# Etschbeijer/GibbsSampling

Measured on NVIDIA B200. Metric: gibbs_window_scores_per_sec, higher is better.
Workload: dtype f64

## Files before the change

### gibbssampling_b200/_abi.py

```python
from __future__ import annotations

import ctypes as C
import os

from . import _build

GIBBS_OK = 0
GIBBS_ERR_ARG = 1
GIBBS_ERR_SYMBOL = 2
GIBBS_ERR_SHORT_SEQ = 3
GIBBS_ERR_CUDA = 4
GIBBS_ERR_NCCL = 5
GIBBS_ERR_NOMEM = 6
GIBBS_ERR_ROULETTE = 7
GIBBS_ERR_UNSUPPORTED = 8

GIBBS_SITE_SAMPLER = 0
GIBBS_MOTIF_SAMPLER = 1
GIBBS_RNG_PHILOX = 0
GIBBS_RNG_INJECTED = 1
GIBBS_BG_FIXED = 0
GIBBS_BG_DATA = 1
GIBBS_MAX_K = 32
PHASE_INIT, PHASE_GREEDY, PHASE_LEFT, PHASE_RIGHT, PHASE_STOCHASTIC, PHASE_MOTIF_GREEDY = 1, 2, 4, 8, 16, 32

EXPORTS = [
    "gibbs_abi_version", "gibbs_last_error", "gibbs_device_count", "gibbs_create", "gibbs_upload",
    "gibbs_destroy", "gibbs_set_stream", "gibbs_num_sequences", "gibbs_set_team_warps", "gibbs_synchronize",
    "gibbs_loo_counts", "gibbs_window_scores", "gibbs_pick_argmax", "gibbs_pick_roulette",
    "gibbs_set_start_ppm", "gibbs_set_start_state", "gibbs_run_device", "gibbs_fetch", "gibbs_run", "gibbs_device_results",
    "gibbs_host_alloc", "gibbs_host_free", "gibbs_measure_smem_bandwidth",
    "gibbs_set_option", "gibbs_fetch_best", "gibbs_fetch_positions", "gibbs_fetch_best_positions",
    "gibbs_set_start_motif_state",
    "gibbs_multi_create", "gibbs_multi_destroy", "gibbs_multi_num_devices", "gibbs_multi_handle",
    "gibbs_multi_run_device", "gibbs_multi_fetch_best",
    "gibbs_batch_create", "gibbs_batch_destroy", "gibbs_batch_run_device", "gibbs_batch_fetch", "gibbs_batch_fetch_best",
]
GIBBS_OPT_INIT_PATH, GIBBS_OPT_EXACT_SCANS, GIBBS_OPT_STAGE2_AT, GIBBS_OPT_STAGE3_AT, GIBBS_OPT_CLUSTER, GIBBS_OPT_MIN_WIDTH = 1, 2, 3, 4, 5, 6
GIBBS_OPT_TILE_ROWS = 7
GIBBS_OPT_SEQ_SWEEPS = 8
GIBBS_INIT_AUTO, GIBBS_INIT_CHAIN, GIBBS_INIT_WIDE, GIBBS_INIT_SMEM, GIBBS_INIT_TILED = 0, 1, 2, 3, 4


class GibbsError(RuntimeError):

    def __init__(self, code: int, msg: str):
        super().__init__(f"[gibbs_status {code}] {msg}")
        self.code = code


class GibbsArgumentError(GibbsError, ValueError):
    """ArgumentNullException / ArgumentException of the reference (fs:24, fs:183)."""


class GibbsSymbolError(GibbsError, IndexError):
    """IndexOutOfRangeException analogue: a symbol the 2-bit tables cannot index (fs:17)."""


class GibbsShortSequenceError(GibbsError, ValueError):
    """InvalidOperationException from Array.take when a sequence is shorter than k (fs:152)."""


class GibbsCudaError(GibbsError):
# ... 126 lines not shown
```

### gibbssampling_b200/csrc/gibbs_api.cu

```cuda
#include "../../include/gibbs_b200.h"
#include "gibbs_kernels.cuh"
#include "gibbs_motif.cuh"
#include "gibbs_motif2.cuh"
#include "gibbs_drift.cuh"
#include "gibbs_batch.cuh"

#include <algorithm>
#include <cmath>
#include <cstdarg>
#include <cstdio>
#include <cstdlib>
#include <cstring>
#include <new>
#include <vector>

namespace gibbs {
#define GIBBS_CHAIN_TU(name) cudaError_t name(const ChainArgs &a, int grid, int smem, cudaStream_t stream)
GIBBS_CHAIN_TU(launch_chain_t1);
GIBBS_CHAIN_TU(launch_chain_t4);
GIBBS_CHAIN_TU(launch_chain_t8);
GIBBS_CHAIN_TU(launch_chain_t16);
GIBBS_CHAIN_TU(launch_chain_masked_t1);
GIBBS_CHAIN_TU(launch_chain_masked_t4);
GIBBS_CHAIN_TU(launch_chain_masked_drift_t1);
// ... 131 lines not shown
    DevBuf<double> start_ppm;
    int32_t start_ppm_k = 0;
    DevBuf<int32_t> basecnt, maskcnt;
    DevBuf<int32_t> ss;
    bool ss_valid = false;
    bool drift_valid = false;
    double drift_pc = 0;
    int32_t drift_alen = 0;
    int32_t gcnt[4] = {0, 0, 0, 0};
    DevBuf<int32_t> ctl, resume, pending;
    int32_t run_extra_launches = 0;
    int32_t team_warps = 0;
    int32_t run_team = 0;
    int sm_count = 0;
    std::vector<int32_t> len_host;
    int32_t start_max_excess = 0;
    int32_t opt_init_path = 0;
    int32_t opt_exact_scans = 0;
    int32_t opt_stage2_at = 4, opt_stage3_at = 1;
    int32_t opt_min_width = -1;
    int32_t opt_seq_sweeps = 1;
    int32_t opt_tile_rows = 0;
    int32_t opt_cluster = 8;
    int32_t cluster_cap[2] = {-1, -1};
    int32_t cluster_cap_n = 0, cluster_cap_rw = 0, cluster_cap_k = 0;
    int32_t run_stages = 0;
    int32_t wt_span = 0, drift_span = 0;
    DevBuf<int32_t> pos2;
    DevBuf<double> sc2;
    int32_t run_m = 1;
    int32_t start_m = 0;
    bool best_valid = false;
    int32_t run_init_path = 0;
    DevBuf<int32_t> win_sites;
    DevBuf<double> win_scores;
    size_t smem_optin = 0;
};

namespace {

int32_t set_device(const gibbs_handle *h) {
    CUDA_TRY(cudaSetDevice(h->device));
    return GIBBS_OK;
}

int32_t check_params(const gibbs_handle *h, const gibbs_params *p) {
    if (!h) return fail(GIBBS_ERR_ARG, "null handle");
    if (!p) return fail(GIBBS_ERR_ARG, "null params");
    if (h->n < 1) return fail(GIBBS_ERR_ARG, "handle holds no sequences");
    if (p->k < 1 || p->k > GIBBS_MAX_K) return fail(GIBBS_ERR_ARG, "motif width k=%d outside 1..%d", p->k, GIBBS_MAX_K);
    if (h->min_len < p->k)
        return fail(GIBBS_ERR_SHORT_SEQ, "a sequence of length %d is shorter than k=%d (Array.take, fs:152)", h->min_len, p->k);
    if (p->alphabet_size < 1) return fail(GIBBS_ERR_ARG, "alphabet_size must be >= 1");
    if (!(p->pseudocount >= 0.0)) return fail(GIBBS_ERR_ARG, "pseudocount must be >= 0");
    if (p->background != GIBBS_BG_FIXED && p->background != GIBBS_BG_DATA) return fail(GIBBS_ERR_ARG, "unknown background mode %d", p->background);
    if (h->has_gap && p->alphabet_size >= 5)
        return fail(GIBBS_ERR_UNSUPPORTED, "sequences hold Gap '-' and alphabet_size = %d includes it: a fifth PWM row is not built "
                                           "(pass alphabet_size = 4 to score Gap like any other non-alphabet symbol)", p->alphabet_size);
    if (p->background == GIBBS_BG_FIXED)
// ... 144 lines not shown
        b.from_list = 0;
        b.pause_below = 0;
        cudaError_t e;
        if (masked && drift) e = team == 4 ? launch_chain_init_masked_drift_t4(b, a.n_chains, smem, h->stream) : launch_chain_init_masked_drift_t1(b, a.n_chains, smem, h->stream);
        else if (masked) e = team == 4 ? launch_chain_init_masked_t4(b, a.n_chains, smem, h->stream) : launch_chain_init_masked_t1(b, a.n_chains, smem, h->stream);
        else if (drift) e = team == 4 ? launch_chain_init_drift_t4(b, a.n_chains, smem, h->stream) : launch_chain_init_drift_t1(b, a.n_chains, smem, h->stream);
        else e = team == 4 ? launch_chain_init_t4(b, a.n_chains, smem, h->stream) : launch_chain_init_t1(b, a.n_chains, smem, h->stream);
        CUDA_TRY(e);
        a.phase_mask &= ~GIBBS_PHASE_INIT;
        h->run_extra_launches += 1;
    }
    return GIBBS_OK;
}

int32_t launch_random_starts_any(gibbs_handle *h, ChainArgs &a, bool drift) {
    switch ((a.k + 1) / 2) {
#define X(KPV) case KPV: return launch_random_starts<KPV>(h, a, drift);
        KP_CASES(X)
#undef X
    default: return fail(GIBBS_ERR_ARG, "unsupported k");
    }
}

template <int KPV>
int32_t launch_chain_kp(gibbs_handle *h, ChainArgs a, bool drift) {
    h->run_extra_launches = 0;
    const bool masked = a.s.mask != nullptr;
    {
        const int32_t rc = launch_random_starts<KPV>(h, a, drift);
        if (rc) return rc;
    }
    const int N = a.s.n, sms = h->sm_count;
    auto fits = [&](int t) { return N >= t && team_smem_bytes(a.s.row_words, t) <= 200 * 1024; };
    struct Stage { int team, pause_below, cluster, min_sweeps; };
    Stage stages[8] = {};
    int n_stages = 0;
    if (masked) {
        stages[n_stages++] = {team_smem_bytes(a.s.row_words, 4) <= 200 * 1024 ? 4 : 1, 0, 0};
    } else if (drift) {
        const int forced = h->team_warps == 16 ? 8 : h->team_warps;
        if (forced != 0) {
            stages[n_stages++] = {forced, 0, 0};
        } else {
            int first = a.n_chains > 2 * sms ? 4 : 8;
            if (first == 8 && !fits(8)) first = 4;
            if (first == 4 && !fits(4)) first = 1;
// ... 25 lines not shown
            if (h->cluster_cap_n != N || h->cluster_cap_rw != a.s.row_words || h->cluster_cap_k != a.k) {
                h->cluster_cap[0] = h->cluster_cap[1] = 0;
                int cap = 0;
                if (launch_chain_cluster4_smem(N, a.s.row_words) <= h->smem_optin &&
                    launch_chain_cluster4(a, 1, h->stream, &cap) == cudaSuccess) h->cluster_cap[0] = cap;
                cap = 0;
                if (launch_chain_cluster8_smem(N, a.s.row_words) <= h->smem_optin &&
                    launch_chain_cluster8(a, 1, h->stream, &cap) == cudaSuccess) h->cluster_cap[1] = cap;
                cudaGetLastError();
                h->cluster_cap_n = N; h->cluster_cap_rw = a.s.row_words; h->cluster_cap_k = a.k;
            }
            if (h->cluster_cap[0] > 0) {
                stages[n_stages - 1].pause_below = h->cluster_cap[0];
                stages[n_stages++] = {16, 0, 4};
                if (h->opt_cluster >= 8 && h->cluster_cap[1] > 0 && h->cluster_cap[1] < h->cluster_cap[0]) {
                    stages[n_stages - 1].pause_below = h->cluster_cap[1];
                    stages[n_stages++] = {16, 0, 8};
                }
            }
        }
    }
    h->run_team = stages[0].team == 1 && n_stages > 1 && stages[0].pause_below == a.n_chains ? 4 : stages[0].team;
    h->run_stages = n_stages;
    CUDA_TRY(h->ctl.reserve(8));
    const int32_t ctl0[8] = {a.n_chains, 0, 0, 0, 0, 0, 0, 0};
    CUDA_TRY(cudaMemcpyAsync(h->ctl.p, ctl0, sizeof ctl0, cudaMemcpyHostToDevice, h->stream));
    a.active = h->ctl.p;
    if (n_stages > 1) {
        CUDA_TRY(h->resume.reserve((size_t)a.n_chains));
        CUDA_TRY(h->pending.reserve((size_t)(n_stages - 1) * (size_t)a.n_chains));
        a.resume = h->resume.p;
    }
    for (int st = 0; st < n_stages; ++st) {
        ChainArgs b = a;
        b.pause_below = stages[st].pause_below;
        b.pause_min_sweeps = stages[st].min_sweeps;
        b.from_list = st > 0;
        {
            const int per_sm = st == 0 ? (a.n_chains + sms - 1) / sms : (stages[st - 1].pause_below + sms - 1) / sms;
            const bool seq_stage = stages[0].team == 1 && stages[0].min_sweeps > 0;
            b.min_width = stages[st].cluster ? stages[st].cluster * 16 : per_sm <= 1 ? stages[st].team
                          : h->opt_min_width >= 1 ? h->opt_min_width : seq_stage ? stages[st].team : 1;
        }
        b.pending_in = st > 0 ? h->pending.p + (size_t)(st - 1) * a.n_chains : nullptr;
        b.pending_in_n = st > 0 ? h->ctl.p + st : nullptr;
        b.pending_out = st + 1 < n_stages ? h->pending.p + (size_t)st * a.n_chains : nullptr;
        b.pending_out_n = st + 1 < n_stages ? h->ctl.p + st + 1 : nullptr;
        const int grid = st == 0 ? a.n_chains : stages[st - 1].pause_below;
        if (stages[st].cluster) {
            CUDA_TRY(stages[st].cluster == 4 ? launch_chain_cluster4(b, grid, h->stream, nullptr) : launch_chain_cluster8(b, grid, h->stream, nullptr));
        } else {
            int32_t rc = launch_team(h, stages[st].team, masked, drift, b, grid);
            if (rc) return rc;
        }
        if (st > 0) h->run_extra_launches += 1;
    }
    return GIBBS_OK;
}

int32_t launch_chain(gibbs_handle *h, const ChainArgs &a, bool drift = false) {
    const int kp = (a.k + 1) / 2;
    switch (kp) {
#define X(KPV) case KPV: return launch_chain_kp<KPV>(h, a, drift);
        KP_CASES(X)
#undef X
    default: return fail(GIBBS_ERR_ARG, "unsupported k");
    }
}

int32_t launch_loo_counts(gibbs_handle *h, const PrimArgs &a) {
    const int kp = (a.k + 1) / 2;
// ... 354 lines not shown
    if (!out) return fail(GIBBS_ERR_ARG, "null out pointer");
    *out = nullptr;
    int ndev = 0;
    cudaError_t e = cudaGetDeviceCount(&ndev);
    if (e != cudaSuccess || ndev < 1) {
        cudaGetLastError();
        return fail(GIBBS_ERR_CUDA, "no CUDA device available (%s); libgibbs_b200 has no CPU fallback",
                    e != cudaSuccess ? cudaGetErrorString(e) : "device count 0");
    }
    if (device < 0 || device >= ndev) return fail(GIBBS_ERR_ARG, "device %d outside 0..%d", device, ndev - 1);
    gibbs_handle *h = new (std::nothrow) gibbs_handle();
    if (!h) return fail(GIBBS_ERR_NOMEM, "host allocation failed");
    h->device = device;
    int32_t rc = set_device(h);
    if (!rc) {
        cudaError_t e2 = cudaStreamCreateWithFlags(&h->stream, cudaStreamNonBlocking);
        if (e2 == cudaSuccess) e2 = cudaEventCreate(&h->ev0);
        if (e2 == cudaSuccess) e2 = cudaEventCreate(&h->ev1);
        if (e2 != cudaSuccess) rc = fail(GIBBS_ERR_CUDA, "stream/event creation: %s", cudaGetErrorString(e2));
        h->own_stream = true;
    }
    if (!rc) {
        cudaError_t e3 = cudaDeviceGetAttribute(&h->sm_count, cudaDevAttrMultiProcessorCount, device);
        int optin = 0;
        if (e3 == cudaSuccess) e3 = cudaDeviceGetAttribute(&optin, cudaDevAttrMaxSharedMemoryPerBlockOptin, device);
        if (e3 != cudaSuccess) rc = fail(GIBBS_ERR_CUDA, "device attribute: %s", cudaGetErrorString(e3));
        h->smem_optin = (size_t)(optin > 0 ? optin : 0);
    }
    if (!rc) rc = upload(h, seqs, offsets, n_seqs);
    if (rc) {
        gibbs_destroy(h);
        return rc;
    }
    *out = h;
    return GIBBS_OK;
}

int32_t gibbs_upload(gibbs_handle *h, const uint8_t *seqs, const int64_t *offsets, int32_t n_seqs) {
    if (!h) return fail(GIBBS_ERR_ARG, "null handle");
    return upload(h, seqs, offsets, n_seqs);
}

int32_t gibbs_destroy(gibbs_handle *h) {
    if (!h) return GIBBS_OK;
    cudaSetDevice(h->device);
    if (h->stream) cudaStreamSynchronize(h->stream);
    h->ascii.release(); h->off.release(); h->packed.release(); h->len.release(); h->flags.release();
    h->mask.release(); h->rowflag.release(); h->symflags.release(); h->wide.release();
    h->wtab.release(); h->prim_sites.release(); h->prim_i32.release(); h->prim_f64.release();
    h->sites.release(); h->hv.release(); h->scores.release(); h->sums.release(); h->uniforms.release();
// ... 589 lines not shown
        if (counts_out) memset(counts_out, 0, (size_t)h->run_k * 4 * sizeof(int32_t));
    }
    if (n_out) *n_out = best < 0 ? 1 : N;
    if (sum_out) *sum_out = sum;
    if (restart_out) *restart_out = best;
    if (stats_out) {
        float ms = 0.f;
        CUDA_TRY(cudaEventElapsedTime(&ms, h->ev0, h->ev1));
        stats_out->site_updates = (int64_t)st[ST_SITE_UPDATES];
        stats_out->window_scores = (int64_t)st[ST_WINDOW_SCORES];
        stats_out->sweeps = (int64_t)st[ST_SWEEPS];
        stats_out->exact_rescans = (int64_t)st[ST_EXACT_RESCANS];
        stats_out->capped_chains = (int64_t)st[ST_CAPPED];
        stats_out->speculative_discards = (int64_t)st[ST_SPECULATED];
        stats_out->kernel_launches = h->run_launches + extra_launches;
        stats_out->fast_path = h->run_fast;
        stats_out->team_warps = h->run_team;
        stats_out->init_path = h->run_init_path;
        stats_out->kernel_ms = (double)ms;
    }
    return GIBBS_OK;
}

int32_t gibbs_set_option(gibbs_handle *h, int32_t option, int32_t value) {
    if (!h) return fail(GIBBS_ERR_ARG, "null handle");
    switch (option) {
    case GIBBS_OPT_INIT_PATH:
        if (value < GIBBS_INIT_AUTO || value > GIBBS_INIT_TILED) return fail(GIBBS_ERR_ARG, "GIBBS_OPT_INIT_PATH takes GIBBS_INIT_AUTO .. GIBBS_INIT_TILED");
        h->opt_init_path = value;
        return GIBBS_OK;
    case GIBBS_OPT_EXACT_SCANS:
        h->opt_exact_scans = value != 0;
        return GIBBS_OK;
    case GIBBS_OPT_MIN_WIDTH:
        if (value < -1 || value > 128) return fail(GIBBS_ERR_ARG, "GIBBS_OPT_MIN_WIDTH takes -1 (automatic) .. 128");
        h->opt_min_width = value;
        return GIBBS_OK;
    case GIBBS_OPT_SEQ_SWEEPS:
        if (value < 0 || value > 3) return fail(GIBBS_ERR_ARG, "GIBBS_OPT_SEQ_SWEEPS takes 0 .. 3");
        h->opt_seq_sweeps = value;
        return GIBBS_OK;
    case GIBBS_OPT_TILE_ROWS:
        if (value < 0) return fail(GIBBS_ERR_ARG, "GIBBS_OPT_TILE_ROWS takes 0 (what fits) or a positive number of sequences");
        h->opt_tile_rows = value;
        return GIBBS_OK;
    case GIBBS_OPT_CLUSTER:
        if (value != 0 && value != 4 && value != 8) return fail(GIBBS_ERR_ARG, "GIBBS_OPT_CLUSTER takes 0, 4 or 8");
        h->opt_cluster = value;
        return GIBBS_OK;
    case GIBBS_OPT_STAGE2_AT:
    case GIBBS_OPT_STAGE3_AT:
        if (value < 1 || value > 16) return fail(GIBBS_ERR_ARG, "hand-over thresholds are 1 .. 16 chains per SM");
        (option == GIBBS_OPT_STAGE2_AT ? h->opt_stage2_at : h->opt_stage3_at) = value;
        if (h->opt_stage3_at > h->opt_stage2_at) h->opt_stage3_at = h->opt_stage2_at;
        return GIBBS_OK;
    default:
        return fail(GIBBS_ERR_ARG, "unknown option %d", option);
    }
}

int32_t gibbs_run(gibbs_handle *h, const gibbs_params *p, int32_t n_chains, int64_t chain_id_base, uint64_t seed,
                  int32_t rng_mode, const double *uniforms, int64_t uniforms_per_chain, int32_t *sites_out,
                  double *scores_out, double *sums_out, int32_t *best_chain_out, int32_t *counts_out,
                  gibbs_run_stats *stats_out) {
    int32_t rc = gibbs_run_device(h, p, n_chains, chain_id_base, seed, rng_mode, uniforms, uniforms_per_chain);
    if (rc) return rc;
    return gibbs_fetch(h, sites_out, scores_out, sums_out, best_chain_out, counts_out, stats_out);
}

struct gibbs_multi {
    std::vector<gibbs_handle *> dev;
// ... 667 lines not shown
```

### gibbssampling_b200/csrc/gibbs_batch.cuh

```cuda
#pragma once
#include "gibbs_kernels.cuh"

namespace gibbs {

struct BatchTable {
    const ChainArgs *sets;
    const int32_t *set_ids;
    const int32_t *chain_off;
    int32_t n;
};

#ifndef GIBBS_BATCH_T4_MIN_BLOCKS
#define GIBBS_BATCH_T4_MIN_BLOCKS 6
#endif
#ifndef GIBBS_BATCH_T4_DRIFT_MIN_BLOCKS
#define GIBBS_BATCH_T4_DRIFT_MIN_BLOCKS 5
#endif
#define GIBBS_BATCH_MIN_BLOCKS(T, DRIFT, INIT_ONLY) \
    (INIT_ONLY ? (T == 1 ? 8 : 4) : T == 1 ? 16 : DRIFT ? GIBBS_BATCH_T4_DRIFT_MIN_BLOCKS : GIBBS_BATCH_T4_MIN_BLOCKS)

template <int KP, int T, bool MASKED, bool DRIFT, bool INIT_ONLY>
static __global__ void __launch_bounds__(32 * T, GIBBS_BATCH_MIN_BLOCKS(T, DRIFT, INIT_ONLY)) chain_batch_kernel(const ChainArgs run, const BatchTable bt) {
    extern __shared__ __align__(128) unsigned char smem_raw[];
    constexpr int THREADS = 32 * T;
// ... 5 lines not shown
        const int g = blockIdx.x;
        int lo = 0, hi = bt.n - 1;
        while (lo < hi) {
            const int mid = (lo + hi + 1) >> 1;
            if (__ldg(bt.chain_off + mid) <= g) lo = mid;
            else hi = mid - 1;
        }
        sa = bt.sets[__ldg(bt.set_ids + lo)];
        sa.seed = run.seed;
        sa.chain_id_base = run.chain_id_base;
        sa.rng_mode = run.rng_mode;
        sa.phase_mask = run.phase_mask;
        sa.max_sweeps = run.max_sweeps;
        sa.min_width = run.min_width;
        sa.stats = run.stats;
        sa.active = nullptr;
        sa.pause_below = 0;
        sa.from_list = 0;
        s_chain = g - __ldg(bt.chain_off + lo);
    }
    __syncthreads();
    const ChainArgs &a = sa;
    const int chain = s_chain;
#include "gibbs_chain_body.inc"
}

static __global__ void __launch_bounds__(32) restart_select_batch_kernel(const double *all_sums, const int32_t *all_sites,
                                                                         const double *all_scores, const int32_t *seq_off, int n_chains,
                                                                         int reps, int32_t *best_out, int32_t *all_win_sites,
                                                                         double *all_win_scores, double *win_sums) {
    const int set = blockIdx.x, lane = threadIdx.x;
    const int o = seq_off[set], N = seq_off[set + 1] - o, NS = N, motif = 0;
    const size_t cells = (size_t)n_chains * o;
    const double *sums = all_sums + (size_t)set * n_chains;
    const int32_t *sites = all_sites + cells;
    const double *scores = all_scores + cells;
    int32_t *out = best_out + set, *win_sites = all_win_sites + o;
    double *win_scores = all_win_scores + o, *win_sum = win_sums + set;
#include "gibbs_restart_select_body.inc"
}

template <int KP>
static __global__ void __launch_bounds__(32) all_counts_batch_kernel(const ChainArgs *sets, const int32_t *seq_off, const int32_t *sites,
                                                                     int k, int32_t *counts_out) {
    __shared__ int32_t total[MAX_COLS * 4];
    __shared__ uint32_t lut[16];
    __shared__ int32_t fix[MAX_COLS];
// ... 10 lines not shown
```

### gibbssampling_b200/csrc/gibbs_chain_body.inc

```
    const TeamSmem S = carve_smem(smem_raw, T);
    const WarpTables WT = warp_tables(S, warp);
    require_aligned_tables(WT);

    const int N = a.s.n, k = a.k;
    int32_t *sites = a.sites + (size_t)chain * N;
    double *hv = a.hv + (size_t)chain * N;
    double *scores = a.scores + (size_t)chain * N;
    const uint64_t chain_uid = (uint64_t)a.chain_id_base + (uint64_t)chain;

    RowRing<R> ring;
    ring.init(S, a.s, 0, tid);
    if (tid < 16) S.lut[tid] = hist_lut_entry(tid);
    team_sync<T>();
    if (warp == 0) ring.fill_span(0u, 0, R, lane);

    unsigned long long st_updates = 0, st_windows = 0, st_slow = 0, st_spec = 0;
    int st_sweeps = 0, capped = 0;
    uint32_t vbase = 0;

    int phase = INIT_ONLY ? PH_INIT : next_phase(PH_GREEDY, a.phase_mask);
    int sweeps_in_phase = 0;
    bool resumed = false, paused = false;
    if (a.from_list) {
        const int r = a.resume[chain];
// ... 156 lines not shown
            if (S.flags[2 * T]) {
                paused = true;
                break;
            }
        }
    }
    if (tid == 0)
        for (int i = 0; i < R; ++i) ring.wait(vbase + (uint32_t)i);
    team_sync<T>();
    if (lane == 0) {
        atomicAdd(a.stats + ST_SITE_UPDATES, st_updates);
        atomicAdd(a.stats + ST_WINDOW_SCORES, st_windows);
        atomicAdd(a.stats + ST_EXACT_RESCANS, st_slow);
        atomicAdd(a.stats + ST_SPECULATED, st_spec);
    }
    if (tid == 0) {
        atomicAdd(a.stats + ST_SWEEPS, (unsigned long long)st_sweeps);
        if (!paused) atomicAdd(a.stats + ST_CAPPED, (unsigned long long)capped);
    }
    if (INIT_ONLY) return;
    if (paused) {
        if (tid == 0) {
            a.resume[chain] = phase | (capped << 7) | (sweeps_in_phase << 8);
            a.pending_out[atomicAdd(a.pending_out_n, 1)] = chain;
        }
        return;
    }

    for (int n = tid; n < N; n += THREADS) {
        const double v = __ldcg(hv + n);
        if (v == v) scores[n] = log2_ref(v);
    }
    team_sync<T>();
    if (tid == 0) {
        double sum = 0.0;
        for (int n = 0; n < N; ++n) sum = __dadd_rn(sum, __ldcg(scores + n));
        a.sums[chain] = sum;
        if (a.active) atomicSub(a.active, 1);
    }
```

### gibbssampling_b200/csrc/gibbs_chain_tu.cu

```cuda
#include "gibbs_kernels.cuh"

#ifndef GIBBS_TU_INIT_ONLY
#define GIBBS_TU_INIT_ONLY 0
#endif
#if !defined(GIBBS_TU_NAME) || !defined(GIBBS_TU_T) || !defined(GIBBS_TU_MASKED) || !defined(GIBBS_TU_DRIFT)
#error "compile with -DGIBBS_TU_NAME=... -DGIBBS_TU_T=... -DGIBBS_TU_MASKED=... -DGIBBS_TU_DRIFT=... (see _build.py)"
#endif

namespace gibbs {

template <int KPV>
static cudaError_t launch_one(const ChainArgs &a, int grid, int smem, cudaStream_t stream) {
    auto kernel = chain_kernel<KPV, GIBBS_TU_T, GIBBS_TU_MASKED != 0, GIBBS_TU_DRIFT != 0, GIBBS_TU_INIT_ONLY != 0>;
    if (smem > 48 * 1024) {
        const cudaError_t e = cudaFuncSetAttribute(kernel, cudaFuncAttributeMaxDynamicSharedMemorySize, smem);
        if (e != cudaSuccess) return e;
    }
    kernel<<<grid, 32 * GIBBS_TU_T, smem, stream>>>(a);
    return cudaGetLastError();
}

cudaError_t GIBBS_TU_NAME(const ChainArgs &a, int grid, int smem, cudaStream_t stream) {
    switch ((a.k + 1) / 2) {
#define X(KPV) case KPV: return launch_one<KPV>(a, grid, smem, stream);
        X(1) X(2) X(3) X(4) X(5) X(6) X(7) X(8) X(9) X(10) X(11) X(12) X(13) X(14) X(15) X(16)
#undef X
    default: return cudaErrorInvalidValue;
    }
}

}
```

### gibbssampling_b200/csrc/gibbs_cluster.cuh

```cuda
#pragma once
#include "gibbs_kernels.cuh"

namespace gibbs {

constexpr int CL_T = 16;

__device__ __forceinline__ uint32_t cluster_ctarank() {
    uint32_t r;
    asm volatile("mov.u32 %0, %%cluster_ctarank;" : "=r"(r));
    return r;
}
__device__ __forceinline__ void cluster_barrier() {
    asm volatile("barrier.cluster.arrive.release.aligned;\n\tbarrier.cluster.wait.acquire.aligned;" ::: "memory");
}
__device__ __forceinline__ uint32_t map_to_rank(const void *smem_ptr, uint32_t rank) {
    uint32_t out;
    asm volatile("mapa.shared::cluster.u32 %0, %1, %2;" : "=r"(out) : "r"(smem_u32(smem_ptr)), "r"(rank));
    return out;
}
__device__ __forceinline__ void st_cluster_u32(uint32_t addr, uint32_t v) {
    asm volatile("st.shared::cluster.u32 [%0], %1;" ::"r"(addr), "r"(v) : "memory");
}
__device__ __forceinline__ void st_cluster_u64(uint32_t addr, uint64_t v) {
    asm volatile("st.shared::cluster.u64 [%0], %1;" ::"r"(addr), "l"(v) : "memory");
// ... 4 lines not shown
__device__ __forceinline__ void cp_async_wait_all() { asm volatile("cp.async.commit_group;\n\tcp.async.wait_group 0;" ::: "memory"); }

template <int C>
__host__ __device__ constexpr int cl_flags_off() { return 704; }
template <int C>
__host__ __device__ constexpr int cl_delta_off() { return cl_flags_off<C>() + 2 * C * CL_T * 4; }
template <int C>
__host__ __device__ constexpr int cl_ctl_off() { return cl_delta_off<C>() + 2 * C * CL_T * 16; }
template <int C>
__host__ __device__ constexpr int cl_tables_off() { return (cl_ctl_off<C>() + 16 + 63) / 64 * 64; }
template <int C>
__host__ __device__ inline size_t cluster_smem_bytes(int n, int row_words) {
    return (size_t)cl_tables_off<C>() + (size_t)CL_T * WARP_TABLE_BYTES + (size_t)CL_T * 2 * row_words * 4 + (size_t)n * 4 * sizeof(WEnt);
}

template <int KP, int C>
static __global__ void __launch_bounds__(32 * CL_T, 1) chain_cluster_kernel(const ChainArgs a) {
    extern __shared__ __align__(128) unsigned char smem_raw[];
    constexpr int T = CL_T, THREADS = 32 * CL_T, GW = C * CL_T;
    const int tid = threadIdx.x, lane = tid & 31, warp = tid >> 5;
    const uint32_t crank = cluster_ctarank();
    const int gw = (int)crank * T + warp;
    const int entry = blockIdx.x / C;
    if (entry >= *a.pending_in_n) return;
    const int chain = a.pending_in[entry];

    const int N = a.s.n, k = a.k, row_words = a.s.row_words;
    int32_t *total = reinterpret_cast<int32_t *>(smem_raw);
    int32_t *fix = reinterpret_cast<int32_t *>(smem_raw + 512);
    uint32_t *lut = reinterpret_cast<uint32_t *>(smem_raw + 640);
    int32_t *flags = reinterpret_cast<int32_t *>(smem_raw + cl_flags_off<C>());
    uint64_t *delta = reinterpret_cast<uint64_t *>(smem_raw + cl_delta_off<C>());
    int32_t *ctl = reinterpret_cast<int32_t *>(smem_raw + cl_ctl_off<C>());
    WarpTables WT;
    {
        unsigned char *b = smem_raw + cl_tables_off<C>() + warp * WARP_TABLE_BYTES;
        WT.wcol = reinterpret_cast<double *>(b);
        WT.ptab = reinterpret_cast<int32_t *>(b + 1024);
        WT.lgcol = reinterpret_cast<int32_t *>(b + 2048);
        WT.counts = reinterpret_cast<int32_t *>(b + 2560);
    }
    require_aligned_tables(WT);
    uint32_t *rows = reinterpret_cast<uint32_t *>(smem_raw + cl_tables_off<C>() + T * WARP_TABLE_BYTES) + warp * 2 * row_words;
    WEnt *wtab_s = reinterpret_cast<WEnt *>(smem_raw + cl_tables_off<C>() + T * WARP_TABLE_BYTES + (size_t)T * 2 * row_words * 4);

    int32_t *sites = a.sites + (size_t)chain * N;
// ... 201 lines not shown
        if (crank == 0 && tid < C) st_cluster_u32(map_to_rank(ctl, (uint32_t)tid), (uint32_t)__shfl_sync((1u << C) - 1u, want_pause, 0));
        cluster_barrier();
        if (ctl[0]) {
            paused = true;
            break;
        }
    }
    cluster_barrier();
    if (lane == 0) {
        atomicAdd(a.stats + ST_SITE_UPDATES, st_updates);
        atomicAdd(a.stats + ST_WINDOW_SCORES, st_windows);
        atomicAdd(a.stats + ST_EXACT_RESCANS, st_slow);
        atomicAdd(a.stats + ST_SPECULATED, st_spec);
    }
    if (crank != 0) return;
    if (tid == 0) {
        atomicAdd(a.stats + ST_SWEEPS, (unsigned long long)st_sweeps);
        if (!paused) atomicAdd(a.stats + ST_CAPPED, (unsigned long long)capped);
    }
    if (paused) {
        if (tid == 0) {
            a.resume[chain] = phase | (capped << 7) | (sweeps_in_phase << 8);
            a.pending_out[atomicAdd(a.pending_out_n, 1)] = chain;
        }
        return;
    }
    for (int n = tid; n < N; n += THREADS) {
        const double v = __ldcg(hv + n);
        if (v == v) scores[n] = log2_ref(v);
    }
    __syncthreads();
    if (tid == 0) {
        double sum = 0.0;
        for (int n = 0; n < N; ++n) sum = __dadd_rn(sum, __ldcg(scores + n));
        a.sums[chain] = sum;
        if (a.active) atomicSub(a.active, 1);
    }
}

}
```

### gibbssampling_b200/csrc/gibbs_device.cuh

```cuda
#pragma once
#include <cuda_runtime.h>
#include <stdint.h>
#include <type_traits>

namespace gibbs {

constexpr unsigned FULL = 0xffffffffu;
constexpr int LG_FRAC_BITS = 11;
constexpr int KEY_IDX_BITS = 8;
constexpr int MAX_COLS = 32;
constexpr double LN2 = 0.6931471805599453;

enum ShiftMode { SHIFT_NONE = 0, SHIFT_LEFT = 1, SHIFT_RIGHT = 2 };
enum StatSlot { ST_SITE_UPDATES = 0, ST_WINDOW_SCORES = 1, ST_SWEEPS = 2, ST_EXACT_RESCANS = 3, ST_CAPPED = 4,
                ST_SPECULATED = 5, ST_NSLOTS = 8 };

struct __align__(16) WEnt {
    double w;
    int32_t lg;
    int32_t pad;
};

struct DeviceSeqs {
    const uint32_t *packed;
// ... 27 lines not shown
    double *sums;
    unsigned long long *stats;
    double cutoff;
    double bg[4];
    const double *ppm_given;
    const double *pvals;
    const int32_t *basecnt;
    const int32_t *maskcnt;
    int32_t gcnt[4];
    double alpha_pc, pc;
    int32_t drift_fast_ok;
    const int32_t *ss;
    int32_t ss_stride;
    int32_t min_width;
    int32_t *active;
    int32_t pause_below;
    int32_t pause_min_sweeps;
    int32_t from_list;
    int32_t *resume;
    const int32_t *pending_in;
    const int32_t *pending_in_n;
    int32_t *pending_out;
    int32_t *pending_out_n;
};

struct WarpTables {
    double *wcol;
    int32_t *ptab;
    int32_t *lgcol;
    int32_t *counts;
};
constexpr int WARP_TABLE_BYTES = 1024 + 1024 + 512 + 512;

struct TeamSmem {
    uint64_t *bar;
    int32_t *total;
    int32_t *flags;
    uint32_t *lut;
    int32_t *fix;
    double *blk_hv;
    int32_t *blk_site;
    int32_t *blk_len;
    unsigned char *warp_tables;
    uint32_t *row0;
};

constexpr int MAX_TEAM = 16;
// ... 732 lines not shown
```

### gibbssampling_b200/csrc/gibbs_kernels.cuh

```cuda
#pragma once
#include "gibbs_device.cuh"
#include "gibbs_drift_dev.cuh"

namespace gibbs {

enum Phase { PH_INIT = 0, PH_GREEDY = 1, PH_LEFT = 2, PH_RIGHT = 3, PH_DONE = 4 };

__device__ __forceinline__ int next_phase(int from, int mask) {
    int ph = from;
    while (ph < PH_DONE && !((mask >> ph) & 1)) ++ph;
    return ph;
}

static __global__ void pack_kernel(const uint8_t *__restrict__ ascii, const int64_t *__restrict__ off, int n, int row_words,
                            uint32_t *__restrict__ packed, uint32_t *__restrict__ mask, int32_t *__restrict__ rowflag,
                            int32_t *__restrict__ len_out, int *flags) {
    const int64_t t = (int64_t)blockIdx.x * blockDim.x + threadIdx.x;
    if (t >= (int64_t)n * row_words) return;
    const int i = (int)(t / row_words), wd = (int)(t % row_words);
    const int64_t o = off[i];
    const int len = (int)(off[i + 1] - o);
    if (wd == 0) len_out[i] = len;
    uint32_t v = 0, m = 0;
    int other = 0;
// ... 510 lines not shown
                build_tables<KP>(WT, WT.counts, false, 0, k, a.wtab, lane);
                double p;
                int w;
                const bool slow = pick_argmax<KP>(WT, own_row, Wn, k, a.fast_ok, lane, p, w);
                if (lane == 0) {
                    a.sites[(size_t)chain * N + n] = w;
                    a.hv[(size_t)chain * N + n] = p;
                }
                st_updates += 1;
                st_windows += (unsigned long long)Wn;
                st_slow += slow ? 1 : 0;
                __syncwarp();
            }
        }
    }
    if (lane == 0) {
        atomicAdd(a.stats + ST_SITE_UPDATES, st_updates);
        atomicAdd(a.stats + ST_WINDOW_SCORES, st_windows);
        atomicAdd(a.stats + ST_EXACT_RESCANS, st_slow);
    }
    if (blockIdx.x == 0 && tid == 0) atomicAdd(a.stats + ST_SWEEPS, (unsigned long long)a.n_chains);
}

template <int KP, int T, bool MASKED = false, bool DRIFT = false, bool INIT_ONLY = false>
static __global__ void __launch_bounds__(32 * T, (INIT_ONLY ? (T == 1 ? 8 : 4) : T == 1 ? 16 : T == 4 ? GIBBS_T4_MIN_BLOCKS : T == 8 ? GIBBS_T8_MIN_BLOCKS : GIBBS_T16_MIN_BLOCKS)) chain_kernel(const ChainArgs a) {
    extern __shared__ __align__(128) unsigned char smem_raw[];
    constexpr int THREADS = 32 * T;
    constexpr int R = (2 * T < 4) ? 4 : 2 * T;
    const int tid = threadIdx.x, lane = tid & 31, warp = tid >> 5;
    int chain = blockIdx.x;
    if (a.from_list) {
        if ((int)blockIdx.x >= *a.pending_in_n) return;
        chain = a.pending_in[blockIdx.x];
    }
#include "gibbs_chain_body.inc"
}

struct PrimArgs {
    DeviceSeqs s;
    const WEnt *wtab;
    const int32_t *sites;
    int32_t heldout;
    int32_t k;
    int32_t fast_ok;
    int32_t *counts_out;
    double *raw_out;
    double *log2_out;
    double *score_out;
    int32_t *site_out;
};

template <int KP>
static __global__ void __launch_bounds__(32) loo_counts_kernel(const PrimArgs a) {
    extern __shared__ __align__(128) unsigned char smem_raw[];
    const int lane = threadIdx.x;
    const TeamSmem S = carve_smem(smem_raw, 1);
    if (lane < 16) S.lut[lane] = hist_lut_entry(lane);
    __syncwarp();
// ... 115 lines not shown
```

### include/gibbs_b200.h

```cpp
#ifndef GIBBS_B200_H
#define GIBBS_B200_H

#include <stddef.h>
#include <stdint.h>

#ifdef __cplusplus
extern "C" {
#endif

#define GIBBS_ABI_VERSION 2
#define GIBBS_MAX_K 32
#define GIBBS_MAX_LEN (1 << 20)

typedef enum gibbs_status {
    GIBBS_OK = 0,
    GIBBS_ERR_ARG = 1,
    GIBBS_ERR_SYMBOL = 2,
    GIBBS_ERR_SHORT_SEQ = 3,
    GIBBS_ERR_CUDA = 4,
    GIBBS_ERR_NCCL = 5,
    GIBBS_ERR_NOMEM = 6,
    GIBBS_ERR_ROULETTE = 7,
    GIBBS_ERR_UNSUPPORTED = 8
} gibbs_status;
// ... 44 lines not shown

typedef struct gibbs_handle gibbs_handle;

int32_t gibbs_abi_version(void);
const char *gibbs_last_error(void);
int32_t gibbs_device_count(void);

int32_t gibbs_create(const uint8_t *seqs, const int64_t *offsets, int32_t n_seqs, int32_t device,
                     gibbs_handle **out);
int32_t gibbs_upload(gibbs_handle *h, const uint8_t *seqs, const int64_t *offsets, int32_t n_seqs);
int32_t gibbs_destroy(gibbs_handle *h);
int32_t gibbs_set_stream(gibbs_handle *h, void *cuda_stream);
int32_t gibbs_num_sequences(const gibbs_handle *h);
int32_t gibbs_set_team_warps(gibbs_handle *h, int32_t warps);
int32_t gibbs_synchronize(gibbs_handle *h);
#define GIBBS_OPT_INIT_PATH 1
#define GIBBS_OPT_EXACT_SCANS 2
#define GIBBS_OPT_STAGE2_AT 3
#define GIBBS_OPT_STAGE3_AT 4
#define GIBBS_OPT_CLUSTER 5
#define GIBBS_OPT_MIN_WIDTH 6
#define GIBBS_OPT_TILE_ROWS 7
#define GIBBS_OPT_SEQ_SWEEPS 8
#define GIBBS_INIT_AUTO 0
#define GIBBS_INIT_CHAIN 1
#define GIBBS_INIT_WIDE 2
#define GIBBS_INIT_SMEM 3
#define GIBBS_INIT_TILED 4
int32_t gibbs_set_option(gibbs_handle *h, int32_t option, int32_t value);

int32_t gibbs_loo_counts(gibbs_handle *h, const int32_t *sites, int32_t heldout, int32_t k,
                         int32_t *counts_out);
int32_t gibbs_window_scores(gibbs_handle *h, const int32_t *sites, int32_t heldout,
                            const gibbs_params *p, double *raw_out, double *log2_out);
int32_t gibbs_pick_argmax(gibbs_handle *h, const int32_t *sites, int32_t heldout,
                          const gibbs_params *p, double *score_out, int32_t *site_out);
int32_t gibbs_pick_roulette(gibbs_handle *h, const int32_t *sites, int32_t heldout,
                            const gibbs_params *p, double u, double *pwms_out, int32_t *site_out);

int32_t gibbs_set_start_ppm(gibbs_handle *h, const double *ppm_or_null, int32_t k);
int32_t gibbs_set_start_state(gibbs_handle *h, int32_t n_chains, const int32_t *sites,
                              const double *scores);
int32_t gibbs_run_device(gibbs_handle *h, const gibbs_params *p, int32_t n_chains,
                         int64_t chain_id_base, uint64_t seed, int32_t rng_mode,
                         const double *uniforms_or_null, int64_t uniforms_per_chain);
int32_t gibbs_fetch(gibbs_handle *h, int32_t *sites_out, double *scores_out, double *sums_out,
// ... 49 lines not shown
```

Before: 443.1 billion.

## Stream paused chains between stages via programmatic dependent launch

Multi-stage chain runs now launch the later stages with programmatic stream serialization. Their blocks spin on a per-slot pending list (pre-filled with -1), so a paused chain is picked up as soon as the previous stage publishes it, instead of waiting for that whole kernel to drain. Each stage counts finished blocks in a done counter, and a shared-memory carveout is computed so that blocks from consecutive stages can be resident together. The aim is to hide the tail of one stage and the launch gap before the next. The cost is polling with nanosleep, extra fences and atomics, and the risk of deadlock or lost occupancy if waiting blocks take SM slots from the producers.

```diff
diff --git a/gibbssampling_b200/_abi.py b/gibbssampling_b200/_abi.py
--- a/gibbssampling_b200/_abi.py
+++ b/gibbssampling_b200/_abi.py
@@ -39,6 +39,7 @@
 GIBBS_OPT_INIT_PATH, GIBBS_OPT_EXACT_SCANS, GIBBS_OPT_STAGE2_AT, GIBBS_OPT_STAGE3_AT, GIBBS_OPT_CLUSTER, GIBBS_OPT_MIN_WIDTH = 1, 2, 3, 4, 5, 6
 GIBBS_OPT_TILE_ROWS = 7
 GIBBS_OPT_SEQ_SWEEPS = 8
+GIBBS_OPT_STREAM_HANDOVER = 9
 GIBBS_INIT_AUTO, GIBBS_INIT_CHAIN, GIBBS_INIT_WIDE, GIBBS_INIT_SMEM, GIBBS_INIT_TILED = 0, 1, 2, 3, 4
 
 
diff --git a/gibbssampling_b200/csrc/gibbs_api.cu b/gibbssampling_b200/csrc/gibbs_api.cu
--- a/gibbssampling_b200/csrc/gibbs_api.cu
+++ b/gibbssampling_b200/csrc/gibbs_api.cu
@@ -177,6 +177,7 @@
     int32_t opt_seq_sweeps = 1;
     int32_t opt_tile_rows = 0;
     int32_t opt_cluster = 8;
+    int32_t opt_stream_handover = 1;
     int32_t cluster_cap[2] = {-1, -1};
     int32_t cluster_cap_n = 0, cluster_cap_rw = 0, cluster_cap_k = 0;
     int32_t run_stages = 0;
@@ -190,6 +191,7 @@
     DevBuf<int32_t> win_sites;
     DevBuf<double> win_scores;
     size_t smem_optin = 0;
+    size_t smem_per_sm = 0;
 };
 
 namespace {
@@ -380,6 +382,18 @@
     }
 }
 
+#ifdef GIBBS_STAGE_TRACE
+static unsigned long long *g_stage_trace = nullptr;
+static cudaError_t stage_trace_buffer(unsigned long long **out, cudaStream_t stream) {
+    if (!g_stage_trace) {
+        const cudaError_t e = cudaMalloc(&g_stage_trace, (1 + 4 * STAGE_TRACE_CAP) * sizeof(unsigned long long));
+        if (e != cudaSuccess) return e;
+    }
+    *out = g_stage_trace;
+    return cudaMemsetAsync(g_stage_trace, 0, sizeof(unsigned long long), stream);
+}
+#endif
+
 template <int KPV>
 int32_t launch_chain_kp(gibbs_handle *h, ChainArgs a, bool drift) {
     h->run_extra_launches = 0;
@@ -451,17 +465,37 @@
     }
     h->run_team = stages[0].team == 1 && n_stages > 1 && stages[0].pause_below == a.n_chains ? 4 : stages[0].team;
     h->run_stages = n_stages;
-    CUDA_TRY(h->ctl.reserve(8));
-    const int32_t ctl0[8] = {a.n_chains, 0, 0, 0, 0, 0, 0, 0};
+    const bool streamed = h->opt_stream_handover != 0 && n_stages > 1;
+    int carveout = cudaSharedmemCarveoutDefault;
+    if (streamed && h->smem_per_sm > 0) {
+        size_t need = 0;
+        for (int st = 0; st < n_stages; ++st) {
+            if (stages[st].cluster) continue;
+            const int t = stages[st].team;
+            const size_t blocks = t == 1 ? 16 : t == 4 ? GIBBS_T4_MIN_BLOCKS : t == 8 ? GIBBS_T8_MIN_BLOCKS : GIBBS_T16_MIN_BLOCKS;
+            need = std::max(need, blocks * ((size_t)team_smem_bytes(a.s.row_words, t) + 1024));
+        }
+        carveout = (int)std::min<size_t>(100, (need * 100 + h->smem_per_sm - 1) / h->smem_per_sm);
+    }
+    CUDA_TRY(h->ctl.reserve(16));
+    const int32_t ctl0[16] = {a.n_chains};
     CUDA_TRY(cudaMemcpyAsync(h->ctl.p, ctl0, sizeof ctl0, cudaMemcpyHostToDevice, h->stream));
     a.active = h->ctl.p;
     if (n_stages > 1) {
         CUDA_TRY(h->resume.reserve((size_t)a.n_chains));
         CUDA_TRY(h->pending.reserve((size_t)(n_stages - 1) * (size_t)a.n_chains));
         a.resume = h->resume.p;
-    }
+        if (streamed)
+            CUDA_TRY(cudaMemsetAsync(h->pending.p, 0xff, (size_t)(n_stages - 1) * a.n_chains * sizeof(int32_t), h->stream));
+    }
+#ifdef GIBBS_STAGE_TRACE
+    CUDA_TRY(stage_trace_buffer(&a.trace, h->stream));
+#endif
     for (int st = 0; st < n_stages; ++st) {
         ChainArgs b = a;
+#ifdef GIBBS_STAGE_TRACE
+        b.trace_stage = st;
+#endif
         b.pause_below = stages[st].pause_below;
         b.pause_min_sweeps = stages[st].min_sweeps;
         b.from_list = st > 0;
@@ -476,6 +510,14 @@
         b.pending_out = st + 1 < n_stages ? h->pending.p + (size_t)st * a.n_chains : nullptr;
         b.pending_out_n = st + 1 < n_stages ? h->ctl.p + st + 1 : nullptr;
         const int grid = st == 0 ? a.n_chains : stages[st - 1].pause_below;
+        if (!stages[st].cluster) {
+            b.smem_carveout = carveout;
+            if (streamed) b.done = h->ctl.p + 8 + st;
+            if (streamed && st > 0 && !stages[st - 1].cluster) {
+                b.prev_done = h->ctl.p + 8 + st - 1;
+                b.prev_grid = st == 1 ? a.n_chains : stages[st - 2].pause_below;
+            }
+        }
         if (stages[st].cluster) {
             CUDA_TRY(stages[st].cluster == 4 ? launch_chain_cluster4(b, grid, h->stream, nullptr) : launch_chain_cluster8(b, grid, h->stream, nullptr));
         } else {
@@ -876,10 +918,12 @@
     }
     if (!rc) {
         cudaError_t e3 = cudaDeviceGetAttribute(&h->sm_count, cudaDevAttrMultiProcessorCount, device);
-        int optin = 0;
+        int optin = 0, per_sm = 0;
         if (e3 == cudaSuccess) e3 = cudaDeviceGetAttribute(&optin, cudaDevAttrMaxSharedMemoryPerBlockOptin, device);
+        if (e3 == cudaSuccess) e3 = cudaDeviceGetAttribute(&per_sm, cudaDevAttrMaxSharedMemoryPerMultiprocessor, device);
         if (e3 != cudaSuccess) rc = fail(GIBBS_ERR_CUDA, "device attribute: %s", cudaGetErrorString(e3));
         h->smem_optin = (size_t)(optin > 0 ? optin : 0);
+        h->smem_per_sm = (size_t)(per_sm > 0 ? per_sm : 0);
     }
     if (!rc) rc = upload(h, seqs, offsets, n_seqs);
     if (rc) {
@@ -1515,6 +1559,18 @@
     return GIBBS_OK;
 }
 
+#ifdef GIBBS_STAGE_TRACE
+extern "C" int64_t gibbs_stage_trace(unsigned long long *out, int64_t cap) {
+    if (!g_stage_trace || cudaDeviceSynchronize() != cudaSuccess) return -1;
+    unsigned long long n = 0;
+    if (cudaMemcpy(&n, g_stage_trace, sizeof n, cudaMemcpyDeviceToHost) != cudaSuccess) return -1;
+    if (n > STAGE_TRACE_CAP) n = STAGE_TRACE_CAP;
+    const size_t m = (size_t)std::min<int64_t>((int64_t)n, cap);
+    if (m && cudaMemcpy(out, g_stage_trace + 1, m * 4 * sizeof n, cudaMemcpyDeviceToHost) != cudaSuccess) return -1;
+    return (int64_t)n;
+}
+#endif
+
 int32_t gibbs_set_option(gibbs_handle *h, int32_t option, int32_t value) {
     if (!h) return fail(GIBBS_ERR_ARG, "null handle");
     switch (option) {
@@ -1540,6 +1596,9 @@
     case GIBBS_OPT_CLUSTER:
         if (value != 0 && value != 4 && value != 8) return fail(GIBBS_ERR_ARG, "GIBBS_OPT_CLUSTER takes 0, 4 or 8");
         h->opt_cluster = value;
+        return GIBBS_OK;
+    case GIBBS_OPT_STREAM_HANDOVER:
+        h->opt_stream_handover = value != 0;
         return GIBBS_OK;
     case GIBBS_OPT_STAGE2_AT:
     case GIBBS_OPT_STAGE3_AT:
diff --git a/gibbssampling_b200/csrc/gibbs_batch.cuh b/gibbssampling_b200/csrc/gibbs_batch.cuh
--- a/gibbssampling_b200/csrc/gibbs_batch.cuh
+++ b/gibbssampling_b200/csrc/gibbs_batch.cuh
@@ -51,7 +51,9 @@
     __syncthreads();
     const ChainArgs &a = sa;
     const int chain = s_chain;
+#define GIBBS_CHAIN_EXIT(paused)
 #include "gibbs_chain_body.inc"
+#undef GIBBS_CHAIN_EXIT
 }
 
 static __global__ void __launch_bounds__(32) restart_select_batch_kernel(const double *all_sums, const int32_t *all_sites,
diff --git a/gibbssampling_b200/csrc/gibbs_chain_body.inc b/gibbssampling_b200/csrc/gibbs_chain_body.inc
--- a/gibbssampling_b200/csrc/gibbs_chain_body.inc
+++ b/gibbssampling_b200/csrc/gibbs_chain_body.inc
@@ -202,8 +202,10 @@
     if (paused) {
         if (tid == 0) {
             a.resume[chain] = phase | (capped << 7) | (sweeps_in_phase << 8);
-            a.pending_out[atomicAdd(a.pending_out_n, 1)] = chain;
-        }
+            __threadfence();
+            st_release_gpu(a.pending_out + atomicAdd(a.pending_out_n, 1), chain);
+        }
+        GIBBS_CHAIN_EXIT(true);
         return;
     }
 
diff --git a/gibbssampling_b200/csrc/gibbs_chain_tu.cu b/gibbssampling_b200/csrc/gibbs_chain_tu.cu
--- a/gibbssampling_b200/csrc/gibbs_chain_tu.cu
+++ b/gibbssampling_b200/csrc/gibbs_chain_tu.cu
@@ -16,8 +16,25 @@
         const cudaError_t e = cudaFuncSetAttribute(kernel, cudaFuncAttributeMaxDynamicSharedMemorySize, smem);
         if (e != cudaSuccess) return e;
     }
-    kernel<<<grid, 32 * GIBBS_TU_T, smem, stream>>>(a);
-    return cudaGetLastError();
+    if (a.smem_carveout != 0) {
+        const cudaError_t e = cudaFuncSetAttribute(kernel, cudaFuncAttributePreferredSharedMemoryCarveout, a.smem_carveout);
+        if (e != cudaSuccess) return e;
+    }
+    if (a.prev_done == nullptr) {
+        kernel<<<grid, 32 * GIBBS_TU_T, smem, stream>>>(a);
+        return cudaGetLastError();
+    }
+    cudaLaunchConfig_t cfg = {};
+    cfg.gridDim = dim3((unsigned)grid, 1, 1);
+    cfg.blockDim = dim3(32 * GIBBS_TU_T, 1, 1);
+    cfg.dynamicSmemBytes = (size_t)smem;
+    cfg.stream = stream;
+    cudaLaunchAttribute attr[1];
+    attr[0].id = cudaLaunchAttributeProgrammaticStreamSerialization;
+    attr[0].val.programmaticStreamSerializationAllowed = 1;
+    cfg.attrs = attr;
+    cfg.numAttrs = 1;
+    return cudaLaunchKernelEx(&cfg, kernel, a);
 }
 
 cudaError_t GIBBS_TU_NAME(const ChainArgs &a, int grid, int smem, cudaStream_t stream) {
diff --git a/gibbssampling_b200/csrc/gibbs_cluster.cuh b/gibbssampling_b200/csrc/gibbs_cluster.cuh
--- a/gibbssampling_b200/csrc/gibbs_cluster.cuh
+++ b/gibbssampling_b200/csrc/gibbs_cluster.cuh
@@ -50,6 +50,9 @@
     const uint32_t crank = cluster_ctarank();
     const int gw = (int)crank * T + warp;
     const int entry = blockIdx.x / C;
+#ifdef GIBBS_STAGE_TRACE
+    const unsigned long long t_start = global_ns();
+#endif
     if (entry >= *a.pending_in_n) return;
     const int chain = a.pending_in[entry];
 
@@ -297,6 +300,9 @@
         if (tid == 0) {
             a.resume[chain] = phase | (capped << 7) | (sweeps_in_phase << 8);
             a.pending_out[atomicAdd(a.pending_out_n, 1)] = chain;
+#ifdef GIBBS_STAGE_TRACE
+            stage_trace(a, chain, true, t_start, t_start);
+#endif
         }
         return;
     }
@@ -310,7 +316,10 @@
         for (int n = 0; n < N; ++n) sum = __dadd_rn(sum, __ldcg(scores + n));
         a.sums[chain] = sum;
         if (a.active) atomicSub(a.active, 1);
-    }
-}
-
-}
+#ifdef GIBBS_STAGE_TRACE
+        stage_trace(a, chain, false, t_start, t_start);
+#endif
+    }
+}
+
+}
diff --git a/gibbssampling_b200/csrc/gibbs_device.cuh b/gibbssampling_b200/csrc/gibbs_device.cuh
--- a/gibbssampling_b200/csrc/gibbs_device.cuh
+++ b/gibbssampling_b200/csrc/gibbs_device.cuh
@@ -73,7 +73,66 @@
     const int32_t *pending_in_n;
     int32_t *pending_out;
     int32_t *pending_out_n;
-};
+    const int32_t *prev_done;
+    int32_t prev_grid;
+    int32_t *done;
+    int32_t smem_carveout;
+#ifdef GIBBS_STAGE_TRACE
+    unsigned long long *trace;
+    int32_t trace_stage;
+#endif
+};
+
+__device__ __forceinline__ int32_t ld_relaxed_gpu(const int32_t *p) {
+    int32_t v;
+    asm volatile("ld.relaxed.gpu.global.b32 %0, [%1];" : "=r"(v) : "l"(p) : "memory");
+    return v;
+}
+__device__ __forceinline__ void fence_acq_rel_gpu() { asm volatile("fence.acq_rel.gpu;" ::: "memory"); }
+__device__ __forceinline__ void st_release_gpu(int32_t *p, int32_t v) {
+    asm volatile("st.release.gpu.global.b32 [%0], %1;" ::"l"(p), "r"(v) : "memory");
+}
+__device__ __forceinline__ void pdl_launch_dependents() { asm volatile("griddepcontrol.launch_dependents;" ::: "memory"); }
+__device__ __forceinline__ void pdl_wait() { asm volatile("griddepcontrol.wait;" ::: "memory"); }
+
+__device__ __forceinline__ int wait_for_paused_chain(const ChainArgs &a, int slot) {
+    unsigned ns = 64;
+    for (;;) {
+        int c = ld_relaxed_gpu(a.pending_in + slot);
+        if (c < 0 && ld_relaxed_gpu(a.prev_done) == a.prev_grid) {
+            fence_acq_rel_gpu();
+            c = ld_relaxed_gpu(a.pending_in + slot);
+            if (c < 0) return -1;
+        }
+        if (c >= 0) {
+            fence_acq_rel_gpu();
+            return c;
+        }
+        __nanosleep(ns);
+        if (ns < 1024) ns *= 2;
+    }
+}
+
+#ifdef GIBBS_STAGE_TRACE
+constexpr unsigned long long STAGE_TRACE_CAP = 1u << 16;
+__device__ __forceinline__ unsigned long long global_ns() {
+    unsigned long long t;
+    asm volatile("mov.u64 %0, %globaltimer;" : "=l"(t));
+    return t;
+}
+__device__ __forceinline__ void stage_trace(const ChainArgs &a, int chain, bool paused, unsigned long long t0, unsigned long long t1) {
+    if (a.trace == nullptr) return;
+    unsigned smid;
+    asm volatile("mov.u32 %0, %smid;" : "=r"(smid));
+    const unsigned long long i = atomicAdd(a.trace, 1ull);
+    if (i >= STAGE_TRACE_CAP) return;
+    unsigned long long *r = a.trace + 1 + 4 * i;
+    r[0] = (unsigned long long)a.trace_stage | (paused ? 256ull : 0ull) | ((unsigned long long)smid << 16) | ((unsigned long long)(chain + 1) << 32);
+    r[1] = t0;
+    r[2] = t1;
+    r[3] = global_ns();
+}
+#endif
 
 struct WarpTables {
     double *wcol;
diff --git a/gibbssampling_b200/csrc/gibbs_kernels.cuh b/gibbssampling_b200/csrc/gibbs_kernels.cuh
--- a/gibbssampling_b200/csrc/gibbs_kernels.cuh
+++ b/gibbssampling_b200/csrc/gibbs_kernels.cuh
@@ -556,6 +556,27 @@
     if (blockIdx.x == 0 && tid == 0) atomicAdd(a.stats + ST_SWEEPS, (unsigned long long)a.n_chains);
 }
 
+__device__ __forceinline__ void stage_exit(const ChainArgs &a, int tid
+#ifdef GIBBS_STAGE_TRACE
+                                           , int chain, bool paused, unsigned long long t_start, unsigned long long t_chain
+#endif
+) {
+    if (a.done != nullptr) {
+        __syncthreads();
+        if (tid == 0) {
+#ifdef GIBBS_STAGE_TRACE
+            stage_trace(a, chain, paused, t_start, t_chain);
+#endif
+            __threadfence();
+            atomicAdd(a.done, 1);
+        }
+    }
+#ifdef GIBBS_STAGE_TRACE
+    else if (tid == 0) stage_trace(a, chain, paused, t_start, t_chain);
+#endif
+    pdl_wait();
+}
+
 template <int KP, int T, bool MASKED = false, bool DRIFT = false, bool INIT_ONLY = false>
 static __global__ void __launch_bounds__(32 * T, (INIT_ONLY ? (T == 1 ? 8 : 4) : T == 1 ? 16 : T == 4 ? GIBBS_T4_MIN_BLOCKS : T == 8 ? GIBBS_T8_MIN_BLOCKS : GIBBS_T16_MIN_BLOCKS)) chain_kernel(const ChainArgs a) {
     extern __shared__ __align__(128) unsigned char smem_raw[];
@@ -563,11 +584,34 @@
     constexpr int R = (2 * T < 4) ? 4 : 2 * T;
     const int tid = threadIdx.x, lane = tid & 31, warp = tid >> 5;
     int chain = blockIdx.x;
+#ifdef GIBBS_STAGE_TRACE
+    const unsigned long long t_start = global_ns();
+#define GIBBS_CHAIN_EXIT(paused) stage_exit(a, tid, chain, paused, t_start, t_chain)
+#else
+#define GIBBS_CHAIN_EXIT(paused) stage_exit(a, tid)
+#endif
+    pdl_launch_dependents();
     if (a.from_list) {
-        if ((int)blockIdx.x >= *a.pending_in_n) return;
-        chain = a.pending_in[blockIdx.x];
+        if (a.prev_done != nullptr) {
+            int32_t *slot = reinterpret_cast<int32_t *>(smem_raw);
+            if (tid == 0) *slot = wait_for_paused_chain(a, blockIdx.x);
+            __syncthreads();
+            chain = *slot;
+            __syncthreads();
+        } else {
+            chain = (int)blockIdx.x < *a.pending_in_n ? a.pending_in[blockIdx.x] : -1;
+        }
+    }
+#ifdef GIBBS_STAGE_TRACE
+    const unsigned long long t_chain = global_ns();
+#endif
+    if (chain < 0) {
+        GIBBS_CHAIN_EXIT(false);
+        return;
     }
 #include "gibbs_chain_body.inc"
+    GIBBS_CHAIN_EXIT(false);
+#undef GIBBS_CHAIN_EXIT
 }
 
 struct PrimArgs {
diff --git a/include/gibbs_b200.h b/include/gibbs_b200.h
--- a/include/gibbs_b200.h
+++ b/include/gibbs_b200.h
@@ -90,6 +90,7 @@
 #define GIBBS_OPT_MIN_WIDTH 6
 #define GIBBS_OPT_TILE_ROWS 7
 #define GIBBS_OPT_SEQ_SWEEPS 8
+#define GIBBS_OPT_STREAM_HANDOVER 9
 #define GIBBS_INIT_AUTO 0
 #define GIBBS_INIT_CHAIN 1
 #define GIBBS_INIT_WIDE 2
```

New measurement: 458.1 billion (median of 6 runs). 3.4% higher.
